# thunlp/ConvDR

Measured on AMD Instinct MI355X. Metric: passages encoded/sec + query x passage IP-scored/sec, 768-d, higher is better.
Workload: dtype bf16

## Files before the change

convdr_amd/csrc/encoder.hip:

```cpp
#include "gemm_launch.hpp"
#include "gemm_ln.hpp"
#include "cls_fold.hpp"

#include "../../include/convdr_hip.h"

namespace convdr {

struct EncBufs {
  int32_t* status;
  int32_t *tok_id, *tok_pos;
  bf16_t *X, *Q, *K, *Vt, *ctx, *Hm, *cls_b, *cls_ctx, *cls_x, *cls_x1;
  float *Y, *cls_y, *cls_f, *head_y;
  float* slab;
  int64_t ldt;
  size_t total;
};

constexpr int64_t SPLITK_MAX_ROWS = 42 * 128;
constexpr int SPLITK_MAX_SPLIT = 4;
static int64_t g_ffn2_splitk = 1;

static EncBufs enc_plan(const convdr_encoder_config* c, int64_t rows, int B, char* base) {
  EncBufs p;
  size_t o = 0;
  auto take = [&](size_t bytes) { size_t at = o; o = align_up(o + bytes, 256); return (char*)((uintptr_t)base + at); };
  const int H = c->hidden, I = c->intermediate;
  const int64_t rs = rows + 128;
  p.ldt = align_up((size_t)rows + 64, 8);
  p.status = (int32_t*)take(256);
  p.tok_id = (int32_t*)take(rs * 4);
  p.tok_pos = (int32_t*)take(rs * 4);
  p.X = (bf16_t*)take(rs * H * 2);
  p.Q = (bf16_t*)take(rs * H * 2);
  p.K = (bf16_t*)take(rs * H * 2);
  p.Vt = (bf16_t*)take((size_t)H * p.ldt * 2);
  p.ctx = (bf16_t*)take(rs * H * 2);
  p.Hm = (bf16_t*)take(rs * I * 2);
  p.Y = (float*)take(rs * H * 4);
  p.slab = rows <= SPLITK_MAX_ROWS ? (float*)take((size_t)SPLITK_MAX_SPLIT * rs * H * 4) : nullptr;
  const int64_t Bp = B + 128;
  p.cls_b = (bf16_t*)take(Bp * H * 2);
  p.cls_ctx = (bf16_t*)take(Bp * H * 2);
  p.cls_x = (bf16_t*)take(Bp * H * 2);
  p.cls_x1 = (bf16_t*)take(Bp * H * 2);
  p.cls_y = (float*)take(Bp * H * 4);
  p.cls_f = (float*)take(Bp * H * 4);
  p.head_y = (float*)take(Bp * (c->out_dim > 0 ? c->out_dim : 1) * 4);
  p.total = o;
  return p;
}

static int64_t g_fused_ln_max_k = 1 << 30;
static int64_t g_hm_blocked = 1;
static int64_t g_fused_ln_min_rows = 128 * 192;
static int64_t g_cls_fold = 1;
static int64_t g_cls_fold_min_rows = CLS_FOLD_MIN_ROWS;

static bool fused_ln_applies(int64_t rows, int H, int K) {
  return H == 768 && rows >= g_fused_ln_min_rows && K % LN_SLICE == 0 && K <= g_fused_ln_max_k;
}
static int gemm_resid_ln(const bf16_t* W, const bf16_t* Wks, const bf16_t* A, int64_t rows, int H, int K, const float* bias,
                         const bf16_t* R, const float* gamma, const float* beta, float eps, float* Yf, bf16_t* X,
                         const char* name, hipStream_t st, bool a_blocked = false, float* slab = nullptr) {
  if (fused_ln_applies(rows, H, K)) {
    static DeviceOnce attr_done;
    if (attr_done.first())
      CONVDR_CHECK_HIP(
          hipFuncSetAttribute((const void*)k_gemm_resid_ln, hipFuncAttributeMaxDynamicSharedMemorySize, LN_SMEM_BYTES));
    GemmLnArgs a{W, A, rows, K, bias, R, gamma, beta, eps, X,
                 K == 768 ? (unsigned long long*)g_gemm_trace_ln : nullptr, Wks, a_blocked ? 1 : 0, 0};
#ifdef CONVDR_ENABLE_TRACE
    static const int dbg_epi = getenv("CONVDR_DBG_SKIP_EPI") ? atoi(getenv("CONVDR_DBG_SKIP_EPI")) : 0;
    a.dbg_skip_epi = dbg_epi == 1;
#endif
    ProfScope prof(name, st);
    hipLaunchKernelGGL(k_gemm_resid_ln, dim3((unsigned)ceil_div64(rows, TileLN::TL)), dim3(512), LN_SMEM_BYTES, st, a);
    CONVDR_CHECK_LAUNCH("k_gemm_resid_ln");
    return 0;
  }
  GemmArgs g{};
  int ns = 1;
  if (slab && g_ffn2_splitk && H == 768 && K >= 2048 && rows <= SPLITK_MAX_ROWS) {
    const int64_t tiles = ceil_div64(rows, 128) * (H / 128), slots = (int64_t)device_cu_count() * 2;
    for (int c = SPLITK_MAX_SPLIT; c >= 2; c >>= 1)
      if (tiles * c <= slots && K % (c * GEMM_BK) == 0) { ns = c; break; }
  }
  if (ns > 1) {
    g.rows = rows; g.W = W; g.X = A; g.N = H; g.K = K; g.k_split_len = K / ns; g.Cf = slab;
    if (int e = launch_gemm<EPI_SLAB_F32>(g, st, name)) return e;
    ProfScope prof("layernorm", st);
    hipLaunchKernelGGL(k_slab_finish_ln<3>, dim3((unsigned)ceil_div64(rows, 4)), dim3(256), 0, st, slab, ns, rows, bias, R, gamma, beta,
                       eps, X);
    CONVDR_CHECK_LAUNCH("k_slab_finish_ln");
    return 0;
  }
  g.rows = rows; g.W = W; g.X = A; g.N = H; g.K = K; g.bias = bias; g.Cf = Yf; g.R = R;
  if (int e = launch_gemm<EPI_RESID_F32>(g, st, name)) return e;
  ProfScope prof("layernorm", st);
  launch_layernorm_bf16(Yf, rows, H, gamma, beta, eps, X, st);
  CONVDR_CHECK_LAUNCH("k_layernorm");
  return 0;
}

static int check_config(const convdr_encoder_config* c) {
  CONVDR_REQUIRE(c->hidden % 128 == 0 && c->hidden <= 1024, "encoder: hidden must be a multiple of 128, <= 1024 (got %d)",
                 c->hidden);
  CONVDR_REQUIRE(c->heads * 64 == c->hidden, "encoder: head_dim must be 64 (hidden=%d heads=%d)", c->hidden, c->heads);
  CONVDR_REQUIRE(c->intermediate % 64 == 0, "encoder: intermediate %% 64 != 0 (%d)", c->intermediate);
  CONVDR_REQUIRE(c->out_dim == 0 || (c->out_dim % 4 == 0 && c->out_dim <= 1024), "encoder: bad out_dim %d", c->out_dim);
  return 0;
}

int encoder_layer_forward(const convdr_encoder_config* c, const convdr_layer_weights* w, const EncBufs& p,
                          const int32_t* cu, const int32_t* lens, int64_t rows, int B, int max_len, float* lse,
                          bool cls_only, hipStream_t st) {
  const int H = c->hidden, I = c->intermediate;
  GemmArgs g{};
  g.rows = rows;
  g.W = (const bf16_t*)w->wqkv; g.X = p.X; g.N = 3 * H; g.K = H; g.bias = w->bqkv;
  g.Qo = p.Q; g.Ko = p.K; g.Vt = p.Vt; g.H = H; g.ldt = p.ldt;
  const bf16_t *xin = p.X, *ctx = p.ctx;
  bf16_t* x1 = p.X;
  int64_t n = rows;
  const bool blk_on = g_hm_blocked != 0;
  const bool ctx_blocked = blk_on && !cls_only && fused_ln_applies(rows, H, H);
  const bool qk_blocked = blk_on && fused_ln_applies(rows, H, H);
  g.qk_blocked = qk_blocked ? 1 : 0;
  if (!cls_only) {
    if (int e = launch_gemm<EPI_QKV>(g, st, "gemm_qkv")) return e;
    AttnArgs a{p.Q, p.K, p.Vt, p.ldt, cu, lens, H, (int64_t)H, p.ctx, lse, 0.125f, (unsigned long long*)g_attn_trace};
    ProfScope prof("attention", st);
    if (ctx_blocked && qk_blocked) {
      hipLaunchKernelGGL((k_attention_fwd<false, true, true>), dim3((max_len + 127) / 128, c->heads, B), dim3(256), ATT_SMEM_BYTES, st, a);
    } else {
      hipLaunchKernelGGL(k_attention_fwd<false>, dim3((max_len + 127) / 128, c->heads, B), dim3(256), ATT_SMEM_BYTES, st, a);
    }
    CONVDR_CHECK_LAUNCH("k_attention_fwd");
  } else {
    hipLaunchKernelGGL(k_gather_cls, dim3((B + 3) / 4), dim3(256), 0, st, cu, B, H, p.X, (const float*)nullptr, p.cls_x,
                       (float*)nullptr);
    CONVDR_CHECK_LAUNCH("k_gather_cls");
    GemmArgs gq{};
    gq.rows = B; gq.W = (const bf16_t*)w->wqkv; gq.X = p.cls_x; gq.N = H; gq.K = H; gq.bias = w->bqkv; gq.Cb = p.Q;
    if (int e = launch_gemm<EPI_BF16>(gq, st, "gemm_qkv")) return e;
    const size_t fold_bytes = (size_t)B * c->heads * H * sizeof(float);
    const bool fold = g_cls_fold != 0 && rows >= g_cls_fold_min_rows && fold_bytes <= (size_t)(rows + 128) * H * 2 && fold_bytes <= (size_t)H * p.ldt * 2;
    if (fold) {
      float *U = (float*)p.K, *Z = (float*)p.Vt;
      const dim3 fgrid((unsigned)((B + FOLD_ROWS - 1) / FOLD_ROWS), (unsigned)c->heads);
      {
        ProfScope prof("gemm_qkv", st);
        hipLaunchKernelGGL(k_cls_key_fold, fgrid, dim3(256), 0, st, p.Q, (const bf16_t*)w->wqkv + (size_t)H * H, B, H, 0.125f, U);
        CONVDR_CHECK_LAUNCH("k_cls_key_fold");
      }
      {
        ProfScope prof("attention", st);
        if (int e = launch_cls_pool(p.X, U, cu, lens, B, H, Z, st)) return e;
      }
      ProfScope prof("gemm_qkv", st);
      hipLaunchKernelGGL(k_cls_value_fold, fgrid, dim3(256), 0, st, Z, (const bf16_t*)w->wqkv + (size_t)2 * H * H, w->bqkv + 2 * H, B, H,
                         p.cls_ctx);
      CONVDR_CHECK_LAUNCH("k_cls_value_fold");
    } else {
      g.W = (const bf16_t*)w->wqkv + (size_t)H * H; g.bias = w->bqkv + H; g.N = 2 * H; g.third0 = 1;
      if (int e = launch_gemm<EPI_QKV>(g, st, "gemm_qkv")) return e;
      AttnArgs a{p.Q, p.K, p.Vt, p.ldt, cu, lens, H, (int64_t)H, p.cls_ctx, nullptr, 0.125f, nullptr};
      ProfScope prof("attention", st);
      if (qk_blocked) hipLaunchKernelGGL((k_attention_fwd<true, false, true>), dim3(1, c->heads, B), dim3(256), ATT_SMEM_BYTES, st, a);
      else hipLaunchKernelGGL(k_attention_fwd<true>, dim3(1, c->heads, B), dim3(256), ATT_SMEM_BYTES, st, a);
      CONVDR_CHECK_LAUNCH("k_attention_fwd<cls>");
    }
    xin = p.cls_x; ctx = p.cls_ctx; x1 = p.cls_x1; n = B;
  }
  if (int e = gemm_resid_ln((const bf16_t*)w->wo, (const bf16_t*)w->wo_ks, ctx, n, H, H, w->bo, xin, w->ln1_g, w->ln1_b, c->ln_eps, p.Y, x1,
                            "gemm_attn_out", st, ctx_blocked))
    return e;
  GemmArgs g2{};
  g2.rows = n; g2.W = (const bf16_t*)w->w1; g2.X = x1; g2.N = I; g2.K = H; g2.bias = w->b1; g2.Cb = p.Hm;
  const bool blocked = blk_on && !cls_only && fused_ln_applies(n, H, I) && I % 256 == 0 && (I / 256) * ceil_div64(n, 256) >= 192;
  if (blocked) {
    if (int e = launch_gemm<EPI_GELU_BLK>(g2, st, "gemm_ffn1")) return e;
    return gemm_resid_ln((const bf16_t*)w->w2, (const bf16_t*)w->w2_ks, p.Hm, n, H, I, w->b2, x1, w->ln2_g, w->ln2_b, c->ln_eps, p.Y,
                         p.X, "gemm_ffn2", st, true);
  }
  if (int e = launch_gemm<EPI_GELU_BF16>(g2, st, "gemm_ffn1")) return e;
  if (cls_only) {
    g2 = GemmArgs{};
    g2.rows = n; g2.W = (const bf16_t*)w->w2; g2.X = p.Hm; g2.N = H; g2.K = I; g2.bias = w->b2; g2.Cf = p.Y; g2.R = x1;
    return launch_gemm<EPI_RESID_F32>(g2, st, "gemm_ffn2");
  }
  return gemm_resid_ln((const bf16_t*)w->w2, (const bf16_t*)w->w2_ks, p.Hm, n, H, I, w->b2, x1, w->ln2_g, w->ln2_b, c->ln_eps, p.Y, p.X, "gemm_ffn2", st,
                       false, p.slab);
}

}

using namespace convdr;

extern "C" size_t convdr_encoder_workspace_bytes(const convdr_encoder_config* cfg, int64_t rows, int B) {
  return enc_plan(cfg, rows, B, nullptr).total;
}

extern "C" int convdr_cast_f32_bf16(const float* x, void* y, int64_t n, convdr_stream_t stream) {
  CONVDR_REQUIRE(n % 4 == 0, "convdr_cast_f32_bf16: n %% 4 != 0 (%lld)", (long long)n);
  if (n == 0) return 0;
  const int64_t n4 = n / 4;
  const unsigned grid = (unsigned)(ceil_div64(n4, 256) < 4096 ? ceil_div64(n4, 256) : 4096);
  hipLaunchKernelGGL(k_cast_f32_bf16, dim3(grid), dim3(256), 0, (hipStream_t)stream, x, (bf16_t*)y, n4);
  CONVDR_CHECK_LAUNCH("k_cast_f32_bf16");
  return 0;
}

namespace convdr {
static int encoder_forward_packed(const convdr_encoder_config* cfg, const convdr_encoder_weights* w, const EncBufs& p,
                                  const int32_t* cu_seqlens, const int32_t* seq_lens, int64_t rows, int B, int max_len,
                                  float* out, hipStream_t st) {
  const int H = cfg->hidden;
  {
    ProfScope prof("embed_ln", st);
    hipLaunchKernelGGL(k_embed_ln, dim3((unsigned)ceil_div64(rows, 4)), dim3(256), 0, st, p.tok_id, p.tok_pos, rows, H,
                       w->word_emb, w->pos_emb, w->type_emb, w->emb_ln_g, w->emb_ln_b, cfg->ln_eps, p.X, DropSite{0u, 0u, 1.f});
    CONVDR_CHECK_LAUNCH("k_embed_ln");
  }
  for (int l = 0; l < cfg->layers; ++l) {
    const convdr_layer_weights* lw = &w->layers[l];
    const bool last = l + 1 == cfg->layers;
    if (int e = encoder_layer_forward(cfg, lw, p, cu_seqlens, seq_lens, rows, B, max_len, nullptr, last && !cfg->pool_mean, st))
      return e;
    if (last && cfg->pool_mean) {
      hipLaunchKernelGGL(k_masked_mean, dim3(B), dim3(256), 0, st, p.X, cu_seqlens, seq_lens, H, p.cls_b,
                         cfg->out_dim > 0 ? p.cls_f : out);
      CONVDR_CHECK_LAUNCH("k_masked_mean");
    } else if (last) {
      float* cls_out = cfg->out_dim > 0 ? p.cls_f : out;
      hipLaunchKernelGGL(k_layernorm, dim3((B + 3) / 4), dim3(256), 0, st, p.Y, (int64_t)B, H, lw->ln2_g, lw->ln2_b,
                         cfg->ln_eps, p.cls_b, cls_out);
      CONVDR_CHECK_LAUNCH("k_layernorm(cls)");
    }
  }
  if (cfg->out_dim > 0) {
    GemmArgs g{};
    g.rows = B; g.W = (const bf16_t*)w->head_w; g.X = p.cls_b; g.N = cfg->out_dim; g.K = H; g.bias = w->head_b;
    g.Cf = p.head_y;
    if (int e = launch_gemm<EPI_F32>(g, st, "gemm_head")) return e;
    hipLaunchKernelGGL(k_layernorm, dim3((B + 3) / 4), dim3(256), 0, st, p.head_y, (int64_t)B, cfg->out_dim,
                       w->head_ln_g, w->head_ln_b, cfg->head_ln_eps, (bf16_t*)nullptr, out);
    CONVDR_CHECK_LAUNCH("k_layernorm(head)");
  }
  return 0;
}
}

extern "C" int convdr_encoder_forward(const convdr_encoder_config* cfg, const convdr_encoder_weights* w,
                                      const void* input_ids, int ids_are_int32, const int64_t* attention_mask, int B, int L,
                                      const int32_t* cu_seqlens, const int32_t* seq_lens, int64_t rows, int max_len,
                                      void* workspace, size_t workspace_bytes, float* out, convdr_stream_t stream) {
  hipStream_t st = (hipStream_t)stream;
  if (int e = check_config(cfg)) return e;
  CONVDR_REQUIRE(B > 0 && L > 0 && rows > 0 && rows % 8 == 0 && max_len > 0 && max_len <= L,
                 "convdr_encoder_forward: bad sizes B=%d L=%d rows=%lld max_len=%d", B, L, (long long)rows, max_len);
  const EncBufs p = enc_plan(cfg, rows, B, (char*)workspace);
  CONVDR_REQUIRE(workspace_bytes >= p.total, "convdr_encoder_forward: workspace too small (%zu < %zu)", workspace_bytes,
                 p.total);
  const int H = cfg->hidden;
  CONVDR_CHECK_HIP(hipMemset2DAsync(p.Vt + rows, p.ldt * 2, 0, (p.ldt - rows) * 2, H, st));
  CONVDR_CHECK_HIP(hipMemsetAsync(p.status, 0, 256, st));
  hipLaunchKernelGGL(k_seq_pack, dim3((B + 3) / 4), dim3(256), 0, st, input_ids, ids_are_int32, attention_mask, seq_lens, B, L, cu_seqlens,
                     cfg->kind, cfg->pad_idx, cfg->max_pos, cfg->vocab, p.tok_id, p.tok_pos, p.status);
  CONVDR_CHECK_LAUNCH("k_seq_pack");
  return encoder_forward_packed(cfg, w, p, cu_seqlens, seq_lens, rows, B, max_len, out, st);
}

extern "C" int convdr_encoder_forward_ragged(const convdr_encoder_config* cfg, const convdr_encoder_weights* w,
                                             const int32_t* tokens, int64_t n_tokens, const int32_t* tok_offsets, int B,
                                             const int32_t* cu_seqlens, const int32_t* seq_lens, int64_t rows, int max_len,
                                             void* workspace, size_t workspace_bytes, float* out, convdr_stream_t stream) {
  hipStream_t st = (hipStream_t)stream;
  if (int e = check_config(cfg)) return e;
  CONVDR_REQUIRE(B > 0 && n_tokens >= B && n_tokens <= INT32_MAX && rows > 0 && rows % 8 == 0 && rows >= n_tokens && max_len > 0 &&
                     max_len <= n_tokens,
                 "convdr_encoder_forward_ragged: bad sizes B=%d n_tokens=%lld rows=%lld max_len=%d", B, (long long)n_tokens,
                 (long long)rows, max_len);
  CONVDR_REQUIRE(tokens != nullptr && tok_offsets != nullptr, "convdr_encoder_forward_ragged: null tokens / tok_offsets");
  const EncBufs p = enc_plan(cfg, rows, B, (char*)workspace);
  CONVDR_REQUIRE(workspace_bytes >= p.total, "convdr_encoder_forward_ragged: workspace too small (%zu < %zu)", workspace_bytes,
                 p.total);
  const int H = cfg->hidden;
  CONVDR_CHECK_HIP(hipMemset2DAsync(p.Vt + rows, p.ldt * 2, 0, (p.ldt - rows) * 2, H, st));
  CONVDR_CHECK_HIP(hipMemsetAsync(p.status, 0, 256, st));
  hipLaunchKernelGGL(k_seq_pack_ragged, dim3((B + 3) / 4), dim3(256), 0, st, tokens, n_tokens, tok_offsets, seq_lens, B, cu_seqlens,
                     cfg->kind, cfg->pad_idx, cfg->max_pos, cfg->vocab, p.tok_id, p.tok_pos, p.status);
  CONVDR_CHECK_LAUNCH("k_seq_pack_ragged");
  return encoder_forward_packed(cfg, w, p, cu_seqlens, seq_lens, rows, B, max_len, out, st);
}

extern "C" int convdr_encoder_debug_layout(const convdr_encoder_config* cfg, int64_t rows, int B, int64_t* out) {
  const EncBufs p = enc_plan(cfg, rows, B, nullptr);
  const void* v[13] = {p.tok_id, p.tok_pos, p.X, p.Q, p.K, p.Vt, p.ctx, p.Hm, p.Y, p.cls_b, p.cls_y, p.cls_f, p.head_y};
  for (int i = 0; i < 13; ++i) out[i] = (int64_t)(size_t)v[i];
  out[13] = p.ldt;
  return 0;
}

namespace convdr {
static __global__ void __launch_bounds__(256) k_pack_kslice(const bf16_t* __restrict__ w, int n, int k, bf16_t* __restrict__ out) {
  const int64_t total = (int64_t)n * (k / 8);
  for (int64_t i = (int64_t)blockIdx.x * blockDim.x + threadIdx.x; i < total; i += (int64_t)gridDim.x * blockDim.x) {
    const int c = (int)(i & 3);
    const int64_t sr = i >> 2;
    const int r = (int)(sr % n), s = (int)(sr / n);
    *(uint4*)(out + i * 8) = *(const uint4*)(w + (int64_t)r * k + s * 32 + c * 8);
  }
}
}

extern "C" int convdr_pack_kslice(const void* w_bf16, int n, int k, void* out, convdr_stream_t stream) {
  CONVDR_REQUIRE(n > 0 && k > 0 && k % 32 == 0, "convdr_pack_kslice: bad shape %d x %d", n, k);
  const int64_t total = (int64_t)n * (k / 8);
  hipLaunchKernelGGL(k_pack_kslice, dim3((unsigned)(ceil_div64(total, 256) < 4096 ? ceil_div64(total, 256) : 4096)), dim3(256), 0,
                     (hipStream_t)stream, (const bf16_t*)w_bf16, n, k, (bf16_t*)out);
  CONVDR_CHECK_LAUNCH("k_pack_kslice");
  return 0;
}

extern "C" int convdr_set_option(const char* name, int64_t value) {
  if (strcmp(name, "fused_ln_min_rows") == 0) {
    g_fused_ln_min_rows = value;
    return 0;
  }
  if (strcmp(name, "hm_blocked") == 0) {
    g_hm_blocked = value;
    return 0;
  }
  if (strcmp(name, "mfma16") == 0) {
    g_mfma16 = value;
    return 0;
  }
  if (strcmp(name, "cls_fold") == 0) {
    g_cls_fold = value;
    return 0;
  }
  if (strcmp(name, "cls_fold_min_rows") == 0) {
    g_cls_fold_min_rows = value;
    return 0;
  }
  if (strcmp(name, "gemm_tile_policy") == 0) {
    g_gemm_tile_policy = value;
    return 0;
  }
  if (strcmp(name, "attn_bwd_fused") == 0) {
    g_attn_bwd_fused = value;
    return 0;
  }
  if (strcmp(name, "embed_bwd_deterministic") == 0) {
    g_embed_bwd_det = value;
    return 0;
  }
  if (strcmp(name, "ip_fused_finish") == 0) {
    convdr::g_ip_fused_finish = value;
    return 0;
  }
  if (strcmp(name, "gelu_gp") == 0) {
    g_gelu_gp = value;
    return 0;
  }
  if (strcmp(name, "ffn2_splitk") == 0) {
    g_ffn2_splitk = value;
    return 0;
  }
  if (strcmp(name, "ln_rows") == 0) {
    g_ln_rows = value;
    return 0;
  }
  if (strcmp(name, "ln_bwd_rows") == 0) {
    g_ln_bwd_rows = value;
    return 0;
  }
  if (strcmp(name, "train_bwd_stop_layer") == 0) {
    g_train_bwd_stop_layer = value;
    return 0;
  }
  if (strcmp(name, "fused_ln_max_k") == 0) {
    g_fused_ln_max_k = value;
    return 0;
  }
  if (strcmp(name, "clock_probe") == 0) {
    g_clock_probe = (void*)(uintptr_t)value;
    g_clock_probe_next = 0;
    return 0;
  }
  if (strcmp(name, "clock_probe_slots") == 0) {
    g_clock_probe_slots = value > 0 ? value : 1;
    return 0;
  }
  if (strcmp(name, "attn_trace") == 0) {
    g_attn_trace = (void*)(uintptr_t)value;
    return 0;
  }
  if (strcmp(name, "gemm_trace_ln") == 0) {
    g_gemm_trace_ln = (void*)(uintptr_t)value;
    return 0;
  }
  if (strcmp(name, "gemm_trace") == 0) {
    g_gemm_trace = (void*)(uintptr_t)value;
    return 0;
  }
  set_error("convdr_set_option: unknown option %s", name);
  return -1;
}
```

convdr_amd/csrc/gemm_ln.hpp:

```cpp
#pragma once
#include "gemm_nt.hpp"

namespace convdr {

using TileLN = TileCfg<4, 2, 6, 2>;
constexpr int LN_SLICE = 32;
constexpr int LN_R_BYTES = TileLN::TR * 64, LN_L_BYTES = TileLN::TL * 64;
constexpr int LN_SMEM_BYTES = 3 * LN_R_BYTES + 2 * LN_L_BYTES;

struct GemmLnArgs {
  const bf16_t* W;
  const bf16_t* A;
  int64_t rows;
  int K;
  const float* bias;
  const bf16_t* R;
  const float *gamma, *beta;
  float eps;
  bf16_t* X;
  unsigned long long* trace;
  const bf16_t* Wks;
  int a_blocked;
  int dbg_skip_epi;
};
#ifdef CONVDR_ENABLE_TRACE
#define CONVDR_LN_TRACE(ph) \
  if (a.trace && threadIdx.x == 0) a.trace[(size_t)blockIdx.x * 16 + (ph)] = __builtin_amdgcn_s_memtime();
#else
#define CONVDR_LN_TRACE(ph)
#endif

constexpr int LN_DMA_WAVES = 8, LN_DMA_FIRST = 0;
constexpr int LN_W_WAVES = 4, LN_W_FIRST = 0;
constexpr int LN_A_WAVES = 4, LN_A_FIRST = 4;
constexpr int LN_A_AUX = 2;

template <int WAVES = LN_DMA_WAVES, int FIRST = LN_DMA_FIRST>
__device__ __forceinline__ StageSrc ln_stage_src(const bf16_t* __restrict__ G, int64_t ld, int64_t row0, int64_t nrows,
                                                  int wave, int lane) {
  StageSrc s;
  wave = wave >= FIRST ? wave - FIRST : 0;
  int64_t bytes = (nrows - row0) * ld * 2;
  bytes = bytes < 0 ? 0 : (bytes > 0xffffffffll ? 0xffffffffll : bytes);
  const uint64_t base = (uint64_t)(G + row0 * ld);
  const uint32_t lo = __builtin_amdgcn_readfirstlane((uint32_t)base);
  const uint32_t hi = __builtin_amdgcn_readfirstlane((uint32_t)(base >> 32));
  const uint32_t nb = __builtin_amdgcn_readfirstlane((uint32_t)bytes);
  s.rsrc = __builtin_amdgcn_make_buffer_rsrc((void*)(((uint64_t)hi << 32) | lo), 0, nb, 0x00020000);
  const int row = wave * 16 + (lane >> 2);
  const int gch = (lane & 3) ^ ((row >> 2) & 3);
  s.voff = (uint32_t)(row * ld * 2) + gch * 16;
  s.round_pitch = __builtin_amdgcn_readfirstlane((uint32_t)(16 * WAVES * ld * 2));
  return s;
}

template <int ROWS, int WAVES = LN_DMA_WAVES, int FIRST = LN_DMA_FIRST, int AUX = 0>
__device__ __forceinline__ void ln_stage32(const StageSrc& s, int ks, char* lds_tile, int wave,
                                           uint32_t slice_stride = LN_SLICE * 2) {
  if (wave < FIRST || wave >= FIRST + WAVES) return;
  wave -= FIRST;
  constexpr int ROUNDS = ROWS / (16 * WAVES);
  static_assert(ROUNDS * 16 * WAVES == ROWS, "rows must be a multiple of 16 x issuing waves");
#pragma unroll
  for (int i = 0; i < ROUNDS; ++i)
    __builtin_amdgcn_raw_ptr_buffer_load_lds(s.rsrc, (lptr_t)(lds_tile + (i * WAVES + wave) * 16 * 64), 16, s.voff,
                                             i * s.round_pitch + ks * slice_stride, 0, AUX);
}

__global__ void __launch_bounds__(512, 2) k_gemm_resid_ln(const GemmLnArgs a) {
  using T = TileLN;
  extern __shared__ __attribute__((aligned(16))) char smem[];
  const WavePos<T> w;
  const int64_t t0 = (int64_t)blockIdx.x * T::TL;
  char* sW = smem;
  char* sA = smem + 3 * LN_R_BYTES;
  GemmAcc<T> acc;
  acc.zero();
  CONVDR_LN_TRACE(0)
  const int nk = a.K / LN_SLICE;
  const int sw = (w.li >> 2) & 3;
  const int offR = (w.wr * T::MT * 32 + w.li) * 64;
  const int offL = (w.wl * T::NT * 32 + w.li) * 64;

  StageSrc srcW = a.Wks ? ln_stage_src<LN_W_WAVES, LN_W_FIRST>(a.Wks, LN_SLICE, 0, (int64_t)T::TR * (a.K / LN_SLICE), w.wave, w.lane)
                        : ln_stage_src<LN_W_WAVES, LN_W_FIRST>(a.W, a.K, 0, T::TR, w.wave, w.lane);
  const uint32_t w_slice_stride = a.Wks ? T::TR * LN_SLICE * 2 : LN_SLICE * 2;
  StageSrc srcA = ln_stage_src<LN_A_WAVES, LN_A_FIRST>(a.A, a.K, t0, a.rows, w.wave, w.lane);
  uint32_t a_slice_stride = LN_SLICE * 2;
  if (a.a_blocked) {
    const int64_t rows32 = (a.rows + 31) & ~(int64_t)31;
    const int64_t blk_elems = (int64_t)(a.K >> 3) * 256;
    int64_t bytes = (rows32 - t0) / 32 * blk_elems * 2;
    bytes = bytes < 0 ? 0 : (bytes > 0xffffffffll ? 0xffffffffll : bytes);
    const uint64_t base = (uint64_t)(a.A + (t0 >> 5) * blk_elems);
    const uint32_t lo = __builtin_amdgcn_readfirstlane((uint32_t)base);
    const uint32_t hi = __builtin_amdgcn_readfirstlane((uint32_t)(base >> 32));
    const uint32_t nb = __builtin_amdgcn_readfirstlane((uint32_t)bytes);
    srcA.rsrc = __builtin_amdgcn_make_buffer_rsrc((void*)(((uint64_t)hi << 32) | lo), 0, nb, 0x00020000);
    const int wv = w.wave >= LN_A_FIRST ? w.wave - LN_A_FIRST : 0;
    const int row = wv * 16 + (w.lane >> 2);
    const int gch = (w.lane & 3) ^ ((row >> 2) & 3);
    srcA.voff = (uint32_t)((row >> 5) * blk_elems * 2 + gch * 512 + (row & 31) * 16);
    srcA.round_pitch = __builtin_amdgcn_readfirstlane((uint32_t)((16 * LN_A_WAVES / 32) * blk_elems * 2));
    a_slice_stride = 4 * 512;
  }
  static_assert((16 * LN_A_WAVES) % 32 == 0 && TileLN::TL % (16 * LN_A_WAVES) == 0, "blocked A staging: rounds of whole 32-token blocks");
  constexpr int LN_W_DPW = T::TR / (16 * LN_W_WAVES);
  const bool w_wave = w.wave >= LN_W_FIRST && w.wave < LN_W_FIRST + LN_W_WAVES;
  ln_stage32<T::TR, LN_W_WAVES, LN_W_FIRST>(srcW, 0, sW, w.wave, w_slice_stride);
  ln_stage32<T::TL, LN_A_WAVES, LN_A_FIRST, LN_A_AUX>(srcA, 0, sA, w.wave, a_slice_stride);
  if (nk > 1) ln_stage32<T::TR, LN_W_WAVES, LN_W_FIRST>(srcW, 1, sW + LN_R_BYTES, w.wave, w_slice_stride);
#ifdef CONVDR_ENABLE_TRACE
#define CONVDR_LN_STEP(i)                                                                                     \
  if (a.trace && kt == 8 + (i) / 5 && w.lane == 0 && blockIdx.x < 256)                                        \
    a.trace[2048 * 16 + blockIdx.x * 64 + w.wave * 8 + (i)] = __builtin_amdgcn_s_memtime();
#else
#define CONVDR_LN_STEP(i)
#endif
  int wslot = 0;
  for (int kt = 0; kt < nk; ++kt) {
    CONVDR_LN_STEP(5)
    CONVDR_LN_STEP(0)
    if (kt + 1 < nk && w_wave) asm volatile("s_waitcnt vmcnt(%0)" ::"n"(LN_W_DPW) : "memory");
    else lds_dma_wait_all();
    CONVDR_LN_STEP(1)
    lds_barrier();
    CONVDR_LN_STEP(2)
    if (kt + 1 < nk) ln_stage32<T::TL, LN_A_WAVES, LN_A_FIRST, LN_A_AUX>(srcA, kt + 1, sA + ((kt + 1) & 1) * LN_L_BYTES, w.wave, a_slice_stride);
    const bool issue_w = kt + 2 < nk;
    char* w_dst = sW + (wslot == 0 ? 2 : wslot - 1) * LN_R_BYTES;
    CONVDR_LN_STEP(3)
    const char* tR = sW + wslot * LN_R_BYTES + offR;
    const char* tL = sA + (kt & 1) * LN_L_BYTES + offL;
    wslot = wslot == 2 ? 0 : wslot + 1;
    {
      constexpr int UNITS = 2 * T::MT;
      static_assert(T::NT == 2, "TileLN: two activation fragments per sub-step");
      const int ch0 = ((0 + w.hi) ^ sw) * 16, ch1 = ((2 + w.hi) ^ sw) * 16;
      bf16x8 fb[2][T::NT], fa[3];
      auto load_a = [&](int u) { fa[u % 3] = *(const bf16x8*)(tR + (u % T::MT) * 32 * 64 + (u < T::MT ? ch0 : ch1)); };
#pragma unroll
      for (int j = 0; j < T::NT; ++j) fb[0][j] = *(const bf16x8*)(tL + j * 32 * 64 + ch0);
      load_a(0);
      load_a(1);
#pragma unroll
      for (int u = 0; u < UNITS; ++u) {
        if (u + 2 < UNITS) load_a(u + 2);
        if (u == 2) {
#pragma unroll
          for (int j = 0; j < T::NT; ++j) fb[1][j] = *(const bf16x8*)(tL + j * 32 * 64 + ch1);
        }
#pragma unroll
        for (int j = 0; j < T::NT; ++j)
          acc.c[u % T::MT][j] = __builtin_amdgcn_mfma_f32_32x32x16_bf16(fa[u % 3], fb[u / T::MT][j], acc.c[u % T::MT][j], 0, 0, 0);
      }
      __builtin_amdgcn_sched_group_barrier(0x100, T::NT + 2, 0);
#pragma unroll
      for (int u = 0; u < UNITS; ++u) {
        if (u + 2 < UNITS) __builtin_amdgcn_sched_group_barrier(0x100, 1, 0);
        if (u == 2) __builtin_amdgcn_sched_group_barrier(0x100, T::NT, 0);
        __builtin_amdgcn_sched_group_barrier(0x008, T::NT, 0);
      }
    }
    if (issue_w) ln_stage32<T::TR, LN_W_WAVES, LN_W_FIRST>(srcW, kt + 2, w_dst, w.wave, w_slice_stride);
    CONVDR_LN_STEP(4)
  }

  if (a.dbg_skip_epi) {
    float s = 0.f;
#pragma unroll
    for (int mt = 0; mt < T::MT; ++mt)
#pragma unroll
      for (int nt = 0; nt < T::NT; ++nt)
#pragma unroll
        for (int r = 0; r < 16; ++r) s += acc.c[mt][nt][r];
    if (s == 12345.678f) a.X[0] = f32_to_bf16(s);
    return;
  }
  CONVDR_LN_TRACE(1)
  __syncthreads();
  float* sBias = (float*)smem;
  float* sGam = sBias + 768;
  float* sBet = sGam + 768;
  float* sRed = sBet + 768;
  float* sStat = sRed + 128 * 8;
  char* sC = smem + 16384;
  const int slot = w.wr * 2 + w.hi;
  const StageSrc srcR = ln_stage_src(a.R, 768, t0, a.rows, w.wave, w.lane);
  const __amdgpu_buffer_rsrc_t dstX = ln_stage_src(a.X, 768, t0, a.rows, w.wave, w.lane).rsrc;
  typedef __attribute__((address_space(3))) u32x2_t lds_u2_t;
  static_assert((16384 & 511) == 0, "the image base must leave bits 4-8 to the swizzle");
  auto img_base = [&](int lrl) { return lds_off(sC) + (uint32_t)(lrl * 1536 + ((lrl & 31) << 4) + w.hi * 8); };
  auto img_at = [&](uint32_t B, int chunk) {
    return (lds_u2_t*)(uintptr_t)((B ^ (uint32_t)((chunk & 31) << 4)) + (uint32_t)((chunk & ~31) << 4));
  };
  auto opaque = [](int x) {
    asm volatile("" : "+v"(x));
    return x;
  };
  CONVDR_LN_TRACE(2)
#pragma unroll
  for (int nt = 0; nt < T::NT; ++nt) {
    if (nt) __syncthreads();
    const int tid_a = opaque((int)threadIdx.x);
    int lr = tid_a / 96, pp = tid_a - lr * 96;
#pragma unroll
    for (int i = 0; i < 12; ++i) {
      const int c = (pp & ~31) | ((pp ^ lr) & 31);
      const int tok = (lr >> 5) * 64 + nt * 32 + (lr & 31);
      __builtin_amdgcn_raw_ptr_buffer_load_lds(srcR.rsrc, (lptr_t)(sC + (i * 512 + w.wave * 64) * 16), 16,
                                               (uint32_t)(tok * 1536 + c * 16), 0, 0, 0);
      pp += 32; lr += 5;
      if (pp >= 96) { pp -= 96; lr += 1; }
    }
    if (nt == 0) {
      for (int i = threadIdx.x; i < 768; i += 512) { sBias[i] = a.bias[i]; sGam[i] = a.gamma[i]; sBet[i] = a.beta[i]; }
      CONVDR_LN_TRACE(8)
    }
    lds_dma_wait_all();
    if (nt == 0) { CONVDR_LN_TRACE(9) }
    __syncthreads();
    if (nt == 0) { CONVDR_LN_TRACE(10) }
    float s = 0.f;
    const uint32_t imgB = img_base(opaque(w.wl * 32 + w.li));
#pragma unroll
    for (int mt = 0; mt < T::MT; ++mt) {
      u32x2_t res[4];
#pragma unroll
      for (int g = 0; g < 4; ++g) res[g] = *img_at(imgB, (w.wr * T::MT + mt) * 4 + g);
#pragma unroll
      for (int g = 0; g < 4; ++g) {
        f32x16& v = acc.c[mt][nt];
        const float4 bv = *(const float4*)(sBias + w.r_base(mt, g));
        const u32x2_t r = res[g];
        v[4 * g + 0] += bv.x + __uint_as_float(r.x << 16);
        v[4 * g + 1] += bv.y + __uint_as_float(r.x & 0xffff0000u);
        v[4 * g + 2] += bv.z + __uint_as_float(r.y << 16);
        v[4 * g + 3] += bv.w + __uint_as_float(r.y & 0xffff0000u);
        s += (v[4 * g + 0] + v[4 * g + 1]) + (v[4 * g + 2] + v[4 * g + 3]);
      }
    }
    sRed[(w.wl * 64 + nt * 32 + w.li) * 8 + slot] = s;
    if (nt == 0) { CONVDR_LN_TRACE(11) }
  }
  CONVDR_LN_TRACE(3)
  __syncthreads();
  CONVDR_LN_TRACE(4)
  if (threadIdx.x < 128) {
    const float* p = sRed + threadIdx.x * 8;
    sStat[threadIdx.x] = (((p[0] + p[1]) + (p[2] + p[3])) + ((p[4] + p[5]) + (p[6] + p[7]))) * (1.f / 768.f);
  }
  __syncthreads();
  float mean[T::NT];
#pragma unroll
  for (int nt = 0; nt < T::NT; ++nt) {
    mean[nt] = sStat[w.wl * 64 + nt * 32 + w.li];
    float q = 0.f;
#pragma unroll
    for (int mt = 0; mt < T::MT; ++mt)
#pragma unroll
      for (int r = 0; r < 16; ++r) {
        const float d = acc.c[mt][nt][r] - mean[nt];
        q += d * d;
      }
    sRed[(w.wl * 64 + nt * 32 + w.li) * 8 + slot] = q;
  }
  CONVDR_LN_TRACE(5)
  __syncthreads();
  if (threadIdx.x < 128) {
    const float* p = sRed + threadIdx.x * 8;
    const float var = (((p[0] + p[1]) + (p[2] + p[3])) + ((p[4] + p[5]) + (p[6] + p[7]))) * (1.f / 768.f);
    sStat[128 + threadIdx.x] = rsqrtf(var + a.eps);
  }
  __syncthreads();
  CONVDR_LN_TRACE(6)
#pragma unroll
  for (int nt = 0; nt < T::NT; ++nt) {
    if (nt) __syncthreads();
    const float rstd = sStat[128 + w.wl * 64 + nt * 32 + w.li];
    const uint32_t imgB = img_base(opaque(w.wl * 32 + w.li));
#pragma unroll
    for (int mt = 0; mt < T::MT; ++mt)
#pragma unroll
      for (int g = 0; g < 4; ++g) {
        const int f = w.r_base(mt, g);
        const float4 gg = *(const float4*)(sGam + f), bb = *(const float4*)(sBet + f);
        const f32x16& v = acc.c[mt][nt];
        u32x2_t o;
        o.x = pack_bf16x2((v[4 * g + 0] - mean[nt]) * rstd * gg.x + bb.x, (v[4 * g + 1] - mean[nt]) * rstd * gg.y + bb.y);
        o.y = pack_bf16x2((v[4 * g + 2] - mean[nt]) * rstd * gg.z + bb.z, (v[4 * g + 3] - mean[nt]) * rstd * gg.w + bb.w);
        *img_at(imgB, (w.wr * T::MT + mt) * 4 + g) = o;
      }
    if (nt == 0) { CONVDR_LN_TRACE(12) }
    __syncthreads();
    if (nt == 0) { CONVDR_LN_TRACE(13) }
    const int tid_s = opaque((int)threadIdx.x);
    int lr = tid_s / 96, pp = tid_s - lr * 96;
#pragma unroll
    for (int i0 = 0; i0 < 12; i0 += 4) {
      u32x4_t v4[4];
#pragma unroll
      for (int j = 0; j < 4; ++j) v4[j] = *(const u32x4_t*)(sC + ((i0 + j) * 512 + tid_s) * 16);
#pragma unroll
      for (int j = 0; j < 4; ++j) {
        const int c = (pp & ~31) | ((pp ^ lr) & 31);
        const int tok = (lr >> 5) * 64 + nt * 32 + (lr & 31);
        __builtin_amdgcn_raw_buffer_store_b128(v4[j], dstX, (uint32_t)(tok * 1536 + c * 16), 0, NT_LN ? 2 : 0);
        pp += 32; lr += 5;
        if (pp >= 96) { pp -= 96; lr += 1; }
      }
    }
    if (nt == 0) { CONVDR_LN_TRACE(14) }
  }
  CONVDR_LN_TRACE(7)
}

}
```

Measured before the change: 47480.

## Add 16x16x32 MFMA variant of fused GEMM+residual+LayerNorm kernel

Adds a new k_gemm_resid_ln_m16 kernel that computes the fused GEMM, bias, residual and LayerNorm using 16x16x32 MFMA fragments. It uses a new LDS swizzle that a static_assert checks to be bank-conflict free, a hand-scheduled mainloop (sched_group_barrier interleaving of ds_reads and MFMAs) and a reworked epilogue with a 16-slot row reduction. The new kernel is enabled by default through the ln_mfma16 option. The change targets higher MFMA throughput and less LDS contention in the fused-LN layers, at the cost of a large amount of new code whose schedule and register pressure (launch bounds 512,2) may not beat the previous 32-wide path.

```diff
diff --git a/convdr_amd/csrc/encoder.hip b/convdr_amd/csrc/encoder.hip
--- a/convdr_amd/csrc/encoder.hip
+++ b/convdr_amd/csrc/encoder.hip
@@ -53,6 +53,7 @@
 static int64_t g_fused_ln_max_k = 1 << 30;
 static int64_t g_hm_blocked = 1;
 static int64_t g_fused_ln_min_rows = 128 * 192;
+static int64_t g_ln_mfma16 = 1;
 static int64_t g_cls_fold = 1;
 static int64_t g_cls_fold_min_rows = CLS_FOLD_MIN_ROWS;
 
@@ -74,6 +75,15 @@
     a.dbg_skip_epi = dbg_epi == 1;
 #endif
     ProfScope prof(name, st);
+    if (g_ln_mfma16) {
+      static DeviceOnce attr16_done;
+      if (attr16_done.first())
+        CONVDR_CHECK_HIP(
+            hipFuncSetAttribute((const void*)k_gemm_resid_ln_m16, hipFuncAttributeMaxDynamicSharedMemorySize, LN_SMEM_BYTES));
+      hipLaunchKernelGGL(k_gemm_resid_ln_m16, dim3((unsigned)ceil_div64(rows, TileLN::TL)), dim3(512), LN_SMEM_BYTES, st, a);
+      CONVDR_CHECK_LAUNCH("k_gemm_resid_ln_m16");
+      return 0;
+    }
     hipLaunchKernelGGL(k_gemm_resid_ln, dim3((unsigned)ceil_div64(rows, TileLN::TL)), dim3(512), LN_SMEM_BYTES, st, a);
     CONVDR_CHECK_LAUNCH("k_gemm_resid_ln");
     return 0;
@@ -336,6 +346,10 @@
     g_mfma16 = value;
     return 0;
   }
+  if (strcmp(name, "ln_mfma16") == 0) {
+    g_ln_mfma16 = value;
+    return 0;
+  }
   if (strcmp(name, "cls_fold") == 0) {
     g_cls_fold = value;
     return 0;
diff --git a/convdr_amd/csrc/gemm_ln.hpp b/convdr_amd/csrc/gemm_ln.hpp
--- a/convdr_amd/csrc/gemm_ln.hpp
+++ b/convdr_amd/csrc/gemm_ln.hpp
@@ -315,4 +315,326 @@
   CONVDR_LN_TRACE(7)
 }
 
-}
+constexpr int ln16_swz(int row) { return (4 - ((row >> 2) & 3)) & 3; }
+
+constexpr bool ln16_frag_read_conflict_free() {
+  for (int g = 0; g < 4; ++g) {
+    unsigned seen = 0;
+    for (int l = 0; l < 64; ++l) {
+      const int m = l & 31;
+      const bool first = m < 4 || (m >= 12 && m < 16) || (m >= 20 && m < 28);
+      if ((l >> 5) != (g >> 1) || first != ((g & 1) == 0)) continue;
+      const int row = l & 15, q = l >> 4;
+      const int slot = ((row * 64 + ((q ^ ln16_swz(row)) << 4)) >> 4) & 15;
+      if ((seen >> slot) & 1u) return false;
+      seen |= 1u << slot;
+    }
+    if (seen != 0xffffu) return false;
+  }
+  return true;
+}
+static_assert(ln16_frag_read_conflict_free(), "16-row fragment read: 16 distinct 16-byte slots in every ds_read_b128 lane group");
+static_assert(ln16_swz(0) == ln16_swz(16) && ln16_swz(5) == ln16_swz(5 + 16 * LN_W_WAVES), "the swizzle term is round-independent");
+
+constexpr int LN16_RED_SLOTS = 16;
+constexpr int LN16_IMG_OFF = 20480;
+static_assert((3 * 768 + 128 * LN16_RED_SLOTS + 256) * 4 <= LN16_IMG_OFF && LN16_IMG_OFF + 64 * 1536 <= LN_SMEM_BYTES, "epilogue LDS");
+
+struct Ln16Src {
+  StageSrc W, A;
+  uint32_t w_slice_stride, a_slice_stride;
+};
+
+__device__ __forceinline__ Ln16Src ln16_sources(const GemmLnArgs& a, int64_t t0, const WavePos<TileLN>& w) {
+  using T = TileLN;
+  Ln16Src s;
+  s.W = a.Wks ? ln_stage_src<LN_W_WAVES, LN_W_FIRST>(a.Wks, LN_SLICE, 0, (int64_t)T::TR * (a.K / LN_SLICE), w.wave, w.lane)
+              : ln_stage_src<LN_W_WAVES, LN_W_FIRST>(a.W, a.K, 0, T::TR, w.wave, w.lane);
+  s.w_slice_stride = a.Wks ? T::TR * LN_SLICE * 2 : LN_SLICE * 2;
+  s.A = ln_stage_src<LN_A_WAVES, LN_A_FIRST>(a.A, a.K, t0, a.rows, w.wave, w.lane);
+  s.a_slice_stride = LN_SLICE * 2;
+  {
+    const int wv = w.wave >= LN_W_FIRST ? w.wave - LN_W_FIRST : 0;
+    const int row = wv * 16 + (w.lane >> 2);
+    const int gch = (w.lane & 3) ^ ln16_swz(row);
+    s.W.voff = (uint32_t)(row * (a.Wks ? LN_SLICE : a.K) * 2) + gch * 16;
+  }
+  const int wv = w.wave >= LN_A_FIRST ? w.wave - LN_A_FIRST : 0;
+  const int row = wv * 16 + (w.lane >> 2);
+  const int gch = (w.lane & 3) ^ ln16_swz(row);
+  s.A.voff = (uint32_t)(row * a.K * 2) + gch * 16;
+  if (a.a_blocked) {
+    const int64_t rows32 = (a.rows + 31) & ~(int64_t)31;
+    const int64_t blk_elems = (int64_t)(a.K >> 3) * 256;
+    int64_t bytes = (rows32 - t0) / 32 * blk_elems * 2;
+    bytes = bytes < 0 ? 0 : (bytes > 0xffffffffll ? 0xffffffffll : bytes);
+    const uint64_t base = (uint64_t)(a.A + (t0 >> 5) * blk_elems);
+    const uint32_t lo = __builtin_amdgcn_readfirstlane((uint32_t)base);
+    const uint32_t hi = __builtin_amdgcn_readfirstlane((uint32_t)(base >> 32));
+    const uint32_t nb = __builtin_amdgcn_readfirstlane((uint32_t)bytes);
+    s.A.rsrc = __builtin_amdgcn_make_buffer_rsrc((void*)(((uint64_t)hi << 32) | lo), 0, nb, 0x00020000);
+    s.A.voff = (uint32_t)((row >> 5) * blk_elems * 2 + gch * 512 + (row & 31) * 16);
+    s.A.round_pitch = __builtin_amdgcn_readfirstlane((uint32_t)((16 * LN_A_WAVES / 32) * blk_elems * 2));
+    s.a_slice_stride = 4 * 512;
+  }
+  return s;
+}
+
+template <int ORDER>
+__device__ __forceinline__ void ln_mainloop_m16(const Ln16Src& s, int nk, char* smem, GemmAcc16<TileLN>& acc,
+                                                const WavePos<TileLN>& w) {
+  using T = TileLN;
+  constexpr int MB = GemmAcc16<T>::MB, NB = GemmAcc16<T>::NB;
+  static_assert(MB == 12 && NB == 4, "TileLN: 12 x 4 blocks per wave");
+  char* sW = smem;
+  char* sA = smem + 3 * LN_R_BYTES;
+  const int r16 = w.lane & 15;
+  const int ch = ((w.lane >> 4) ^ ln16_swz(r16)) * 16;
+  const int offR = (w.wr * T::MT * 32 + r16) * 64 + ch;
+  const int offL = (w.wl * T::NT * 32 + r16) * 64 + ch;
+  constexpr int LN_W_DPW = T::TR / (16 * LN_W_WAVES);
+  const bool w_wave = w.wave >= LN_W_FIRST && w.wave < LN_W_FIRST + LN_W_WAVES;
+  ln_stage32<T::TR, LN_W_WAVES, LN_W_FIRST>(s.W, 0, sW, w.wave, s.w_slice_stride);
+  ln_stage32<T::TL, LN_A_WAVES, LN_A_FIRST, LN_A_AUX>(s.A, 0, sA, w.wave, s.a_slice_stride);
+  if (nk > 1) ln_stage32<T::TR, LN_W_WAVES, LN_W_FIRST>(s.W, 1, sW + LN_R_BYTES, w.wave, s.w_slice_stride);
+  int wslot = 0;
+  for (int kt = 0; kt < nk; ++kt) {
+    if (kt + 1 < nk && w_wave) asm volatile("s_waitcnt vmcnt(%0)" ::"n"(LN_W_DPW) : "memory");
+    else lds_dma_wait_all();
+    lds_barrier();
+    if (kt + 1 < nk) ln_stage32<T::TL, LN_A_WAVES, LN_A_FIRST, LN_A_AUX>(s.A, kt + 1, sA + ((kt + 1) & 1) * LN_L_BYTES, w.wave, s.a_slice_stride);
+    const bool issue_w = kt + 2 < nk;
+    char* w_dst = sW + (wslot == 0 ? 2 : wslot - 1) * LN_R_BYTES;
+    const char* tR = sW + wslot * LN_R_BYTES + offR;
+    const char* tL = sA + (kt & 1) * LN_L_BYTES + offL;
+    wslot = wslot == 2 ? 0 : wslot + 1;
+    {
+      bf16x8 fb[NB], fa[3];
+      auto load_a = [&](int u) { fa[u % 3] = *(const bf16x8*)(tR + u * 16 * 64); };
+      auto load_b = [&](int j) { fb[j] = *(const bf16x8*)(tL + j * 16 * 64); };
+      auto mm = [&](int u, int j) { acc.c[u][j] = mfma_16x16x32<false>(fa[u % 3], fb[j], acc.c[u][j]); };
+      if constexpr (ORDER == 0) {
+#pragma unroll
+        for (int j = 0; j < NB; ++j) load_b(j);
+        load_a(0);
+        load_a(1);
+#pragma unroll
+        for (int u = 0; u < MB; ++u) {
+          if (u + 2 < MB) load_a(u + 2);
+#pragma unroll
+          for (int j = 0; j < NB; ++j) mm(u, j);
+        }
+        __builtin_amdgcn_sched_group_barrier(0x100, NB + 2, 0);
+#pragma unroll
+        for (int u = 0; u < MB; ++u) {
+          if (u + 2 < MB) __builtin_amdgcn_sched_group_barrier(0x100, 1, 0);
+          __builtin_amdgcn_sched_group_barrier(0x008, NB, 0);
+        }
+      } else {
+        load_b(0); load_b(1);
+        load_a(0); load_a(1);
+        if constexpr (ORDER == 1) { load_b(2); load_b(3); }
+        mm(0, 0); mm(0, 1);
+        if constexpr (ORDER == 2) { load_b(2); load_b(3); }
+        mm(1, 0); mm(1, 1);
+        load_a(2);
+        mm(0, 2); mm(0, 3);
+        load_a(3);
+        mm(1, 2); mm(1, 3);
+#pragma unroll
+        for (int u = 2; u < MB; ++u) {
+          if (u + 2 < MB) load_a(u + 2);
+#pragma unroll
+          for (int j = 0; j < NB; ++j) mm(u, j);
+        }
+        __builtin_amdgcn_sched_group_barrier(0x100, 4, 0);
+        if constexpr (ORDER == 1) {
+          __builtin_amdgcn_sched_group_barrier(0x100, 2, 0);
+          __builtin_amdgcn_sched_group_barrier(0x008, 4, 0);
+        } else {
+          __builtin_amdgcn_sched_group_barrier(0x008, 2, 0);
+          __builtin_amdgcn_sched_group_barrier(0x100, 2, 0);
+          __builtin_amdgcn_sched_group_barrier(0x008, 2, 0);
+        }
+        __builtin_amdgcn_sched_group_barrier(0x100, 1, 0);
+        __builtin_amdgcn_sched_group_barrier(0x008, 2, 0);
+        __builtin_amdgcn_sched_group_barrier(0x100, 1, 0);
+        __builtin_amdgcn_sched_group_barrier(0x008, 2, 0);
+#pragma unroll
+        for (int u = 2; u < MB; ++u) {
+          if (u + 2 < MB) __builtin_amdgcn_sched_group_barrier(0x100, 1, 0);
+          __builtin_amdgcn_sched_group_barrier(0x008, NB, 0);
+        }
+      }
+    }
+    if (issue_w) ln_stage32<T::TR, LN_W_WAVES, LN_W_FIRST>(s.W, kt + 2, w_dst, w.wave, s.w_slice_stride);
+  }
+}
+constexpr int LN16_ORDER = 1;
+
+__global__ void __launch_bounds__(512, 2) k_gemm_resid_ln_m16(const GemmLnArgs a) {
+  using T = TileLN;
+  constexpr int MB = GemmAcc16<T>::MB, NB = GemmAcc16<T>::NB;
+  extern __shared__ __attribute__((aligned(16))) char smem[];
+  const WavePos<T> w;
+  const int64_t t0 = (int64_t)blockIdx.x * T::TL;
+  GemmAcc16<T> acc;
+  acc.zero();
+  CONVDR_LN_TRACE(0)
+  {
+    const Ln16Src src = ln16_sources(a, t0, w);
+    ln_mainloop_m16<LN16_ORDER>(src, a.K / LN_SLICE, smem, acc, w);
+  }
+  if (a.dbg_skip_epi) {
+    float s = 0.f;
+#pragma unroll
+    for (int i = 0; i < MB; ++i)
+#pragma unroll
+      for (int j = 0; j < NB; ++j)
+#pragma unroll
+        for (int r = 0; r < 4; ++r) s += acc.c[i][j][r];
+    if (s == 12345.678f) a.X[0] = f32_to_bf16(s);
+    return;
+  }
+  CONVDR_LN_TRACE(1)
+  __syncthreads();
+  float* sBias = (float*)smem;
+  float* sGam = sBias + 768;
+  float* sBet = sGam + 768;
+  float* sRed = sBet + 768;
+  float* sStat = sRed + 128 * LN16_RED_SLOTS;
+  char* sC = smem + LN16_IMG_OFF;
+  const int q = w.lane >> 4, t16 = w.lane & 15;
+  const int slot = w.wr * 4 + q;
+  const int f0 = w.wr * T::MT * 32 + 4 * q;
+  const StageSrc srcR = ln_stage_src(a.R, 768, t0, a.rows, w.wave, w.lane);
+  const __amdgpu_buffer_rsrc_t dstX = ln_stage_src(a.X, 768, t0, a.rows, w.wave, w.lane).rsrc;
+  typedef __attribute__((address_space(3))) u32x2_t lds_u2_t;
+  static_assert((LN16_IMG_OFF & 511) == 0, "the image base must leave bits 4-8 to the swizzle");
+  auto img_base = [&](int lrl) {
+    return (lds_off(sC) + (uint32_t)(lrl * 1536 + ((lrl & 31) << 4) + (q & 1) * 8)) ^ (uint32_t)((q >> 1) << 4);
+  };
+  auto img_at = [&](uint32_t B, int chunk) {
+    return (lds_u2_t*)(uintptr_t)((B ^ (uint32_t)((chunk & 31) << 4)) + (uint32_t)((chunk & ~31) << 4));
+  };
+  auto opaque = [](int x) {
+    asm volatile("" : "+v"(x));
+    return x;
+  };
+  CONVDR_LN_TRACE(2)
+#pragma unroll
+  for (int h = 0; h < 2; ++h) {
+    if (h) __syncthreads();
+    const int tid_a = opaque((int)threadIdx.x);
+    int lr = tid_a / 96, pp = tid_a - lr * 96;
+#pragma unroll
+    for (int i = 0; i < 12; ++i) {
+      const int c = (pp & ~31) | ((pp ^ lr) & 31);
+      const int tok = (lr >> 5) * 64 + h * 32 + (lr & 31);
+      __builtin_amdgcn_raw_ptr_buffer_load_lds(srcR.rsrc, (lptr_t)(sC + (i * 512 + w.wave * 64) * 16), 16,
+                                               (uint32_t)(tok * 1536 + c * 16), 0, 0, 0);
+      pp += 32; lr += 5;
+      if (pp >= 96) { pp -= 96; lr += 1; }
+    }
+    if (h == 0) {
+      for (int i = threadIdx.x; i < 768; i += 512) { sBias[i] = a.bias[i]; sGam[i] = a.gamma[i]; sBet[i] = a.beta[i]; }
+    }
+    lds_dma_wait_all();
+    __syncthreads();
+#pragma unroll
+    for (int jj = 0; jj < 2; ++jj) {
+      const int j = 2 * h + jj;
+      float s = 0.f;
+      const uint32_t imgB = img_base(opaque(w.wl * 32 + 16 * jj + t16));
+#pragma unroll
+      for (int i0 = 0; i0 < MB; i0 += 4) {
+        u32x2_t res[4];
+#pragma unroll
+        for (int g = 0; g < 4; ++g) res[g] = *img_at(imgB, w.wr * 24 + 2 * (i0 + g));
+#pragma unroll
+        for (int g = 0; g < 4; ++g) {
+          f32x4& v = acc.c[i0 + g][j];
+          const float4 bv = *(const float4*)(sBias + f0 + 16 * (i0 + g));
+          const u32x2_t r = res[g];
+          v[0] += bv.x + __uint_as_float(r.x << 16);
+          v[1] += bv.y + __uint_as_float(r.x & 0xffff0000u);
+          v[2] += bv.z + __uint_as_float(r.y << 16);
+          v[3] += bv.w + __uint_as_float(r.y & 0xffff0000u);
+          s += (v[0] + v[1]) + (v[2] + v[3]);
+        }
+      }
+      sRed[(w.wl * 64 + 16 * j + t16) * LN16_RED_SLOTS + slot] = s;
+    }
+  }
+  CONVDR_LN_TRACE(3)
+  __syncthreads();
+  CONVDR_LN_TRACE(4)
+  auto sum16 = [](const float* p) {
+    return ((((p[0] + p[1]) + (p[2] + p[3])) + ((p[4] + p[5]) + (p[6] + p[7]))) +
+            (((p[8] + p[9]) + (p[10] + p[11])) + ((p[12] + p[13]) + (p[14] + p[15]))));
+  };
+  if (threadIdx.x < 128) sStat[threadIdx.x] = sum16(sRed + threadIdx.x * LN16_RED_SLOTS) * (1.f / 768.f);
+  __syncthreads();
+  float mean[NB];
+#pragma unroll
+  for (int j = 0; j < NB; ++j) {
+    mean[j] = sStat[w.wl * 64 + 16 * j + t16];
+    float qs = 0.f;
+#pragma unroll
+    for (int i = 0; i < MB; ++i)
+#pragma unroll
+      for (int r = 0; r < 4; ++r) {
+        const float d = acc.c[i][j][r] - mean[j];
+        qs += d * d;
+      }
+    sRed[(w.wl * 64 + 16 * j + t16) * LN16_RED_SLOTS + slot] = qs;
+  }
+  CONVDR_LN_TRACE(5)
+  __syncthreads();
+  if (threadIdx.x < 128) {
+    const float var = sum16(sRed + threadIdx.x * LN16_RED_SLOTS) * (1.f / 768.f);
+    sStat[128 + threadIdx.x] = rsqrtf(var + a.eps);
+  }
+  __syncthreads();
+  CONVDR_LN_TRACE(6)
+#pragma unroll
+  for (int h = 0; h < 2; ++h) {
+    if (h) __syncthreads();
+#pragma unroll
+    for (int jj = 0; jj < 2; ++jj) {
+      const int j = 2 * h + jj;
+      const float rstd = sStat[128 + w.wl * 64 + 16 * j + t16];
+      const uint32_t imgB = img_base(opaque(w.wl * 32 + 16 * jj + t16));
+#pragma unroll
+      for (int i = 0; i < MB; ++i) {
+        const int f = f0 + 16 * i;
+        const float4 gg = *(const float4*)(sGam + f), bb = *(const float4*)(sBet + f);
+        const f32x4& v = acc.c[i][j];
+        u32x2_t o;
+        o.x = pack_bf16x2((v[0] - mean[j]) * rstd * gg.x + bb.x, (v[1] - mean[j]) * rstd * gg.y + bb.y);
+        o.y = pack_bf16x2((v[2] - mean[j]) * rstd * gg.z + bb.z, (v[3] - mean[j]) * rstd * gg.w + bb.w);
+        *img_at(imgB, w.wr * 24 + 2 * i) = o;
+      }
+    }
+    __syncthreads();
+    const int tid_s = opaque((int)threadIdx.x);
+    int lr = tid_s / 96, pp = tid_s - lr * 96;
+#pragma unroll
+    for (int i0 = 0; i0 < 12; i0 += 4) {
+      u32x4_t v4[4];
+#pragma unroll
+      for (int jv = 0; jv < 4; ++jv) v4[jv] = *(const u32x4_t*)(sC + ((i0 + jv) * 512 + tid_s) * 16);
+#pragma unroll
+      for (int jv = 0; jv < 4; ++jv) {
+        const int c = (pp & ~31) | ((pp ^ lr) & 31);
+        const int tok = (lr >> 5) * 64 + h * 32 + (lr & 31);
+        __builtin_amdgcn_raw_buffer_store_b128(v4[jv], dstX, (uint32_t)(tok * 1536 + c * 16), 0, NT_LN ? 2 : 0);
+        pp += 32; lr += 5;
+        if (pp >= 96) { pp -= 96; lr += 1; }
+      }
+    }
+  }
+  CONVDR_LN_TRACE(7)
+}
+
+}
```

After: 48350, median of 6. 1.8% higher.
